# 3dv-casia/PanoVLM

Hardware: AMD Instinct MI355X
Metric: M residual+Jacobian evals/sec (point-to-plane, 64k pts/scan) (higher is better)
Workload: dtype f64

## Files before the change

panovlm_amd/csrc/pvlm_eval.hip:

```cpp
#include <algorithm>
#include <cmath>
#include <limits>

#include "pvlm_functors.h"
#include "pvlm_internal.h"

using namespace pvlm_dev;

#ifndef PVLM_NT_LOADS
#define PVLM_NT_LOADS 1
#endif
#ifndef PVLM_GLOBAL_LOADS
#define PVLM_GLOBAL_LOADS 1
#endif
typedef double pvlm_dbl2 __attribute__((ext_vector_type(2)));
#if PVLM_GLOBAL_LOADS
typedef const __attribute__((address_space(1))) pvlm_dbl2* pvlm_col_ptr;
#else
typedef const pvlm_dbl2* pvlm_col_ptr;
#endif
#ifndef PVLM_NT_LOADS_MATERIALISE
#define PVLM_NT_LOADS_MATERIALISE 0
#endif
__device__ __forceinline__ const double* at_byte(const double* base, unsigned bytes) {
  return reinterpret_cast<const double*>(reinterpret_cast<const char*>(base) + bytes);
}
template <bool NT>
__device__ __forceinline__ double2 stream_load2(const double* p) {
  pvlm_col_ptr q = (pvlm_col_ptr)(p);
  const pvlm_dbl2 v = NT ? __builtin_nontemporal_load(q) : *q;
  return make_double2(v.x, v.y);
}
struct pvlm_plane_args {
  const uint16_t* idx;
  const int64_t* pair_idx0;
  const int64_t* chunk_plane0;
  const double* tab;
  const double* const* pair_ptab;
  const int* order;
};
template <bool NT>
__device__ __forceinline__ unsigned stream_load_runs(const uint16_t* base, unsigned row) {
#if PVLM_GLOBAL_LOADS
  typedef const __attribute__((address_space(1))) unsigned* ptr;
#else
  typedef const unsigned* ptr;
#endif
  ptr q = (ptr)(reinterpret_cast<const char*>(base) + 2u * row);
  return NT ? __builtin_nontemporal_load(q) : *q;
}
template <bool NT>
__device__ __forceinline__ uint2 stream_load_words(const uint16_t* base, unsigned row) {
  typedef unsigned pvlm_u2 __attribute__((ext_vector_type(2)));
#if PVLM_GLOBAL_LOADS
  typedef const __attribute__((address_space(1))) pvlm_u2* ptr;
#else
  typedef const pvlm_u2* ptr;
#endif
  ptr q = (ptr)(reinterpret_cast<const char*>(base) + 4u * row);
  const pvlm_u2 v = NT ? __builtin_nontemporal_load(q) : *q;
  return make_uint2(v.x, v.y);
}
__device__ __forceinline__ double table_load(const double* base, unsigned bytes) {
#if PVLM_GLOBAL_LOADS
  typedef const __attribute__((address_space(1))) double* ptr;
#else
  typedef const double* ptr;
#endif
  return *(ptr)(reinterpret_cast<const char*>(base) + bytes);
}
#ifndef PVLM_NT_STORES
#define PVLM_NT_STORES 0
#endif
__device__ __forceinline__ void stream_store2(double2* p, double2 v) {
#if PVLM_NT_STORES
  pvlm_dbl2 w; w.x = v.x; w.y = v.y;
  __builtin_nontemporal_store(w, reinterpret_cast<pvlm_dbl2*>(p));
#else
  *p = v;
#endif
}
__device__ __forceinline__ void stream_store1(double* p, double v) {
#if PVLM_NT_STORES
  __builtin_nontemporal_store(v, p);
#else
  *p = v;
#endif
}


#ifndef PVLM_PREFETCH
#define PVLM_PREFETCH -1
#endif
#ifndef PVLM_FUSED_WAVES
#define PVLM_FUSED_WAVES 2
#endif
#ifndef PVLM_FUSED_WAVES_7COL
#define PVLM_FUSED_WAVES_7COL 4
#endif
#ifndef PVLM_FUSED_WAVES_WAVEFORM
#define PVLM_FUSED_WAVES_WAVEFORM 3
#endif

__global__ void k_pose_table(int n, const double* __restrict__ aa, const double* __restrict__ t, double* __restrict__ tab) {
  const int i = blockIdx.x * blockDim.x + threadIdx.x;
  if (i >= n) return;
  const double x = aa[3 * i], y = aa[3 * i + 1], z = aa[3 * i + 2];
  const double th2 = x * x + y * y + z * z;
  double* o = tab + (size_t)i * PVLM_POSE_TAB;
  double R[9];
  if (th2 > 2.220446049250313e-16) {
    const double th = sqrt(th2);
    const double wx = x / th, wy = y / th, wz = z / th;
    const double c = cos(th), s = sin(th), k = 1.0 - c;
    R[0] = c + wx * wx * k;      R[1] = wx * wy * k - wz * s; R[2] = wy * s + wx * wz * k;
    R[3] = wz * s + wx * wy * k; R[4] = c + wy * wy * k;      R[5] = -wx * s + wy * wz * k;
    R[6] = -wy * s + wx * wz * k; R[7] = wx * s + wy * wz * k; R[8] = c + wz * wz * k;
  } else {
    R[0] = 1; R[1] = -z; R[2] = y; R[3] = z; R[4] = 1; R[5] = -x; R[6] = -y; R[7] = x; R[8] = 1;
  }
  double A, B;
  if (th2 > 1e-6) {
    const double th = sqrt(th2);
    A = (1.0 - cos(th)) / th2;
    B = (th - sin(th)) / (th2 * th);
  } else {
    A = 0.5 - th2 * (1.0 / 24.0) + th2 * th2 * (1.0 / 720.0);
    B = (1.0 / 6.0) - th2 * (1.0 / 120.0) + th2 * th2 * (1.0 / 5040.0);
  }
  const double J[9] = {1.0 + B * (x * x - th2), -A * z + B * x * y,       A * y + B * x * z,
                       A * z + B * x * y,       1.0 + B * (y * y - th2), -A * x + B * y * z,
                       -A * y + B * x * z,      A * x + B * y * z,        1.0 + B * (z * z - th2)};
#pragma unroll
  for (int k = 0; k < 9; ++k) { o[k] = R[k]; o[9 + k] = J[k]; }
  o[18] = t[3 * i]; o[19] = t[3 * i + 1]; o[20] = t[3 * i + 2];
}

__global__ void k_pair_table(int P, const int* __restrict__ ref, const int* __restrict__ nei, int n_poses,
                             const double* __restrict__ pose, double* __restrict__ tab) {
  const int p = blockIdx.x * blockDim.x + threadIdx.x;
  if (p >= P) return;
  const int ir = ref[p], in = nei[p];
  double* o = tab + (size_t)p * PVLM_PAIR_TAB;
  if (ir >= n_poses || in >= n_poses) {
    for (int k = 0; k < PVLM_PAIR_TAB; ++k) o[k] = __longlong_as_double(0x7ff8000000000000LL);
    return;
  }
  const double* a = pose + (size_t)ir * PVLM_POSE_TAB;
  const double* b = pose + (size_t)in * PVLM_POSE_TAB;
  double R[9];
#pragma unroll
  for (int i = 0; i < 3; ++i)
#pragma unroll
    for (int j = 0; j < 3; ++j) R[i * 3 + j] = a[i * 3] * b[j * 3] + a[i * 3 + 1] * b[j * 3 + 1] + a[i * 3 + 2] * b[j * 3 + 2];
#pragma unroll
  for (int k = 0; k < 9; ++k) o[k] = R[k];
#pragma unroll
  for (int i = 0; i < 3; ++i) {
    o[9 + i] = a[18 + i] - (R[i * 3] * b[18] + R[i * 3 + 1] * b[19] + R[i * 3 + 2] * b[20]);
    o[12 + i] = a[18 + i];
  }
#pragma unroll
  for (int k = 0; k < 9; ++k) o[15 + k] = a[9 + k];
#pragma unroll
  for (int i = 0; i < 3; ++i)
#pragma unroll
    for (int j = 0; j < 3; ++j) o[24 + i * 3 + j] = -(R[i * 3] * b[9 + j] + R[i * 3 + 1] * b[9 + 3 + j] + R[i * 3 + 2] * b[9 + 6 + j]);
}

template <int KIND, bool NORM, int NCOLS>
__global__ __launch_bounds__(256) void k_eval_materialise(const double* const* __restrict__ pair_cols,
                                                          const int64_t* __restrict__ pair_stride,
                                                          const int64_t* __restrict__ out_start,
                                                          const int* __restrict__ blk_pair, const int* __restrict__ blk_chunk,
                                                          int chunk_rows, const double* __restrict__ pair_tab, double weight,
                                                          double* __restrict__ r_out, double* __restrict__ J_out, int blk0, int64_t row0) {
  const int bi = blockIdx.x + blk0;
  const int p = blk_pair[bi];
  const double* __restrict__ cols = pair_cols[p];
  const int64_t n_dev = pair_stride[p];
  const int64_t o0 = out_start[p] - row0;
  const int64_t len = out_start[p + 1] - out_start[p];
  const int64_t lo = (int64_t)blk_chunk[bi] * chunk_rows;
  const int64_t hi = min(len, lo + (int64_t)chunk_rows);
  double T[PVLM_PAIR_TAB];
#pragma unroll
  for (int k = 0; k < PVLM_PAIR_TAB; ++k) T[k] = pair_tab[(size_t)p * PVLM_PAIR_TAB + k];
  __shared__ __attribute__((aligned(16))) double stage[4][128 * 12];
  const int lane = threadIdx.x & 63, wv = threadIdx.x >> 6;
  const double* Jl = T + 15; const double* Mn = T + 24; const double* R = T;
  const int64_t n_it = (hi - lo + 511) / 512;
  for (int64_t it = 0; it < n_it; ++it) {
    const int64_t j = lo + it * 512 + 2 * (int64_t)threadIdx.x;
    if (j < hi) {
      double2 v[NCOLS];
#pragma unroll
      for (int c = 0; c < NCOLS; ++c) v[c] = stream_load2<PVLM_NT_LOADS_MATERIALISE != 0>(cols + (size_t)c * n_dev + j);
#pragma unroll
      for (int h = 0; h < 2; ++h) {
        if (j + h >= hi) break;
        double rec[NCOLS];
#pragma unroll
        for (int c = 0; c < NCOLS; ++c) rec[c] = h ? v[c].y : v[c].x;
        Wrench w;
        eval_wrench<KIND, NORM>(rec, T, weight, w);
        stream_store1(r_out + o0 + j + h, w.r);
        if (J_out) {
          double Jr[12];
#pragma unroll
          for (int k = 0; k < 3; ++k) {
            Jr[k] = w.c[0] * Jl[k] + w.c[1] * Jl[3 + k] + w.c[2] * Jl[6 + k];
            Jr[3 + k] = w.g[k];
            Jr[6 + k] = w.c[0] * Mn[k] + w.c[1] * Mn[3 + k] + w.c[2] * Mn[6 + k];
            Jr[9 + k] = -(w.g[0] * R[k] + w.g[1] * R[3 + k] + w.g[2] * R[6 + k]);
          }
          double2* dst = reinterpret_cast<double2*>(&stage[wv][(2 * lane + h) * 12]);
#pragma unroll
          for (int k = 0; k < 6; ++k) dst[k] = make_double2(Jr[2 * k], Jr[2 * k + 1]);
        }
      }
    }
    if (J_out) {
      __builtin_amdgcn_wave_barrier();
      const int64_t row0 = lo + it * 512 + (int64_t)wv * 128;
      const int64_t rows = min((int64_t)128, hi - row0);
      if (rows > 0) {
        double2* gdst = reinterpret_cast<double2*>(J_out + (size_t)(o0 + row0) * 12);
        const double2* src = reinterpret_cast<const double2*>(&stage[wv][0]);
        const int n2 = (int)rows * 6;
#pragma unroll
        for (int t = 0; t < 12; ++t) {
          const int e = t * 64 + lane;
          if (e < n2) stream_store2(gdst + e, src[e]);
        }
      }
      __builtin_amdgcn_wave_barrier();
    }
  }
}

template <int KIND, bool NORM, int NCOLS, int W>
__global__ __launch_bounds__(256) void k_eval_wrench(const double* const* __restrict__ pair_cols, const int64_t* __restrict__ pair_stride,
                                                     const int64_t* __restrict__ out_start, const int* __restrict__ blk_pair,
                                                     const int* __restrict__ blk_chunk, int chunk_rows, const double* __restrict__ pair_tab,
                                                     double weight, double* __restrict__ w_out, int blk0, int64_t row0) {
  const int bi = blockIdx.x + blk0;
  const int p = blk_pair[bi];
  const double* __restrict__ cols = pair_cols[p];
  const int64_t n_dev = pair_stride[p];
  const int64_t o0 = out_start[p] - row0;
  const int64_t len = out_start[p + 1] - out_start[p];
  const int64_t lo = (int64_t)blk_chunk[bi] * chunk_rows;
  const int64_t hi = min(len, lo + (int64_t)chunk_rows);
  double T[15];
#pragma unroll
  for (int k = 0; k < 15; ++k) T[k] = pair_tab[(size_t)p * PVLM_PAIR_TAB + k];
  __shared__ double stage[4][128 * W];
  const int lane = threadIdx.x & 63, wv = threadIdx.x >> 6;
  const int64_t n_it = (hi - lo + 511) / 512;
  for (int64_t it = 0; it < n_it; ++it) {
    const int64_t j = lo + it * 512 + 2 * (int64_t)threadIdx.x;
    if (j < hi) {
      double2 v[NCOLS];
#pragma unroll
      for (int c = 0; c < NCOLS; ++c) v[c] = stream_load2<PVLM_NT_LOADS_MATERIALISE != 0>(cols + (size_t)c * n_dev + j);
#pragma unroll
      for (int h = 0; h < 2; ++h) {
        if (j + h >= hi) break;
        double rec[NCOLS];
#pragma unroll
        for (int c = 0; c < NCOLS; ++c) rec[c] = h ? v[c].y : v[c].x;
        Wrench w;
        eval_wrench<KIND, NORM>(rec, T, weight, w);
        double* dst = &stage[wv][(2 * lane + h) * W];
        if (W == 7) { dst[0] = w.r; dst[1] = w.c[0]; dst[2] = w.c[1]; dst[3] = w.c[2]; dst[4] = w.g[0]; dst[5] = w.g[1]; dst[6] = w.g[2]; }
        else { dst[0] = w.r; dst[1] = w.g[0]; dst[2] = w.g[1]; dst[3] = w.g[2]; }
      }
    }
    __builtin_amdgcn_wave_barrier();
    const int64_t r0 = lo + it * 512 + (int64_t)wv * 128;
    const int64_t rows = min((int64_t)128, hi - r0);
    if (rows > 0) {
      double* g = w_out + (size_t)(o0 + r0) * W;
      const int n = (int)rows * W;
#pragma unroll
      for (int t = 0; t < 2 * W; ++t) {
        const int e = t * 64 + lane;
        if (e < n) stream_store1(g + e, stage[wv][e]);
      }
    }
    __builtin_amdgcn_wave_barrier();
  }
}

__device__ __forceinline__ double wave_sum(double x) {
#pragma unroll
  for (int off = 32; off > 0; off >>= 1) x += __shfl_down(x, off, 64);
  return x;
}

template <int KIND, bool NORM, int NCOLS, int LOSS>
__device__ __forceinline__ void accumulate_row(const double* rec, const double* T, double weight, double loss_a, double a2, double mh_a2, double* acc) {
  Wrench w;
  eval_wrench<KIND, NORM>(rec, T, weight, w);
  const double s = w.r * w.r;
  double rho1 = 1.0, half_rho = 0.5 * s;
  if (LOSS == PVLM_LOSS_HUBER) {
    const double rr = fabs(w.r);
    const bool out = s > a2;
    const double inv = fast_rcp(out ? rr : 1.0);
    rho1 = out ? fmax(std::numeric_limits<double>::min(), loss_a * inv) : 1.0;
    half_rho = out ? fma(loss_a, rr, mh_a2) : half_rho;
  }
  const double vv[6] = {w.c[0], w.c[1], w.c[2], w.g[0], w.g[1], w.g[2]};
  int q = 0;
#pragma unroll
  for (int a = 0; a < 6; ++a) {
    const double wa = rho1 * vv[a];
#pragma unroll
    for (int b = a; b < 6; ++b) acc[q++] += wa * vv[b];
    acc[21 + a] += wa * w.r;
  }
  acc[27] += half_rho;
}

template <int N>
__device__ __forceinline__ double wave_transpose_sum(const double (&a)[N], int lane) {
  static_assert(N <= 32, "at most 32 values");
  double v[32];
#pragma unroll
  for (int k = 0; k < 32; ++k) v[k] = k < N ? a[k] : 0.0;
#pragma unroll
  for (int half = 16; half >= 1; half >>= 1) {
    const bool up = (lane & (2 * half)) != 0;
#pragma unroll
    for (int k = 0; k < half; ++k) {
      const double keep = up ? v[half + k] : v[k];
      const double send = up ? v[k] : v[half + k];
      v[k] = keep + __shfl_xor(send, 2 * half, 64);
    }
  }
  return v[0] + __shfl_xor(v[0], 1, 64);
}

template <int KIND, bool NORM, int NCOLS, int LOSS, bool PR, bool PT>
__global__ __launch_bounds__(256, (NCOLS == 7 ? PVLM_FUSED_WAVES_7COL : PVLM_FUSED_WAVES)) void k_eval_fused(const double* const* __restrict__ pair_cols,
                                                    const int64_t* __restrict__ pair_stride,
                                                    const int64_t* __restrict__ out_start,
                                                    const int* __restrict__ blk_pair, const int* __restrict__ blk_chunk,
                                                    int chunk_rows, const double* __restrict__ pair_tab, double weight,
                                                    double loss_a, double* __restrict__ partials, pvlm_plane_args pr) {
  static_assert(!PR || NCOLS == 7, "plane runs: the 7-column kinds only");
  static_assert(!PT || PR, "the point table: on top of the plane runs only");
  const int slot = (PT && pr.order) ? pr.order[blockIdx.x] : (int)blockIdx.x;
  if (PT && slot < 0) return;
  constexpr int NS = PR ? 3 : NCOLS;
  const int p = blk_pair[slot];
  const double* __restrict__ cols = pair_cols[p];
  const int64_t n_dev = pair_stride[p];
  const int64_t len = out_start[p + 1] - out_start[p];
  const int64_t lo = (int64_t)blk_chunk[slot] * chunk_rows;
  const int64_t hi = min(len, lo + (int64_t)chunk_rows);
  double T[15];
#pragma unroll
  for (int k = 0; k < 15; ++k) T[k] = pair_tab[(size_t)p * PVLM_PAIR_TAB + k];
  double acc[PVLM_PARTIAL];
#pragma unroll
  for (int k = 0; k < PVLM_PARTIAL; ++k) acc[k] = 0.0;
  const double a2 = uniform_sgpr(loss_a * loss_a), mh_a2 = uniform_sgpr(-0.5 * a2);
  constexpr bool kPrefetch = !PT && (PVLM_PREFETCH >= 0 ? (PVLM_PREFETCH != 0) : (KIND == PVLM_POINT2PLANE_METER || KIND == PVLM_POINT2LINE_METER));
  const double* colb[NS];
#pragma unroll
  for (int c = 0; c < NS; ++c) colb[c] = PT ? pr.pair_ptab[p] + (size_t)c * PVLM_POINT_TAB_STRIDE : cols + (size_t)c * n_dev + lo;
  const uint16_t* runb = nullptr;
  const double* tabb = nullptr;
  if (PR) { runb = pr.idx + (PT ? 2 : 1) * (pr.pair_idx0[p] + lo); tabb = pr.tab + 4 * pr.chunk_plane0[slot]; }
  const unsigned span = hi > lo ? (unsigned)(hi - lo) : 0u;
  const unsigned span8 = 8u * span;
  unsigned o = 16u * threadIdx.x;
  double2 nx[NS];
  unsigned nx_runs = 0, nx_qs = 0;
  auto load_words = [&](unsigned row) {
    if (PT) { const uint2 w = stream_load_words<PVLM_NT_LOADS != 0>(runb, row); nx_runs = w.x; nx_qs = w.y; }
    else nx_runs = stream_load_runs<PVLM_NT_LOADS != 0>(runb, row);
  };
  if (PR && o < span8) load_words(o >> 3);
  if (kPrefetch && o < span8) {
#pragma unroll
    for (int c = 0; c < NS; ++c) nx[c] = stream_load2<PVLM_NT_LOADS != 0>(at_byte(colb[c], o));
  }
  for (; o < span8; o += 4096) {
    double2 v[NS];
    const unsigned runs = nx_runs, qs = nx_qs;
    const unsigned o_next = o + 4096 < span8 ? o + 4096 : o;
    if (kPrefetch) {
#pragma unroll
      for (int c = 0; c < NS; ++c) v[c] = nx[c];
      if (PR) load_words(o_next >> 3);
      if (o + 4096 < span8) {
#pragma unroll
        for (int c = 0; c < NS; ++c) nx[c] = stream_load2<PVLM_NT_LOADS != 0>(at_byte(colb[c], o + 4096));
      }
    } else {
#ifdef PVLM_EXP_SKIP
#pragma unroll
      for (int c = 0; c < NS; ++c) v[c] = *reinterpret_cast<const double2*>(colb[c < NS - PVLM_EXP_SKIP ? c : 0] + (o >> 3));
#else
      if (PT) {
        const unsigned q0 = 8u * (qs & 0xffffu), q1 = 8u * (qs >> 16);
#pragma unroll
        for (int c = 0; c < NS; ++c) v[c] = make_double2(table_load(colb[c], q0), table_load(colb[c], q1));
      } else {
#pragma unroll
        for (int c = 0; c < NS; ++c) v[c] = stream_load2<PVLM_NT_LOADS != 0>(at_byte(colb[c], o));
      }
#endif
    }
    double2 pl[2][2];
    if (PR) {
#pragma unroll
      for (int h = 0; h < 2; ++h) {
        const unsigned at = 32u * (h ? runs >> 16 : runs & 0xffffu);
        pl[h][0] = stream_load2<false>(at_byte(tabb, at));
        pl[h][1] = stream_load2<false>(at_byte(tabb, at + 16u));
      }
      if (!kPrefetch) load_words(o_next >> 3);
    }
#pragma unroll
    for (int h = 0; h < 2; ++h) {
      if (o + 8u * h >= span8) break;
      double rec[NCOLS];
#pragma unroll
      for (int c = 0; c < NS; ++c) rec[c] = h ? v[c].y : v[c].x;
      if (PR) { rec[3] = pl[h][0].x; rec[4] = pl[h][0].y; rec[5] = pl[h][1].x; rec[6] = pl[h][1].y; }
      accumulate_row<KIND, NORM, NCOLS, LOSS>(rec, T, weight, loss_a, a2, mh_a2, acc);
    }
  }
  __shared__ double red[4][PVLM_PARTIAL];
  const int lane = threadIdx.x & 63, wv = threadIdx.x >> 6;
  {
    const double s = wave_transpose_sum<PVLM_PARTIAL>(acc, lane);
    if (!(lane & 1) && (lane >> 1) < PVLM_PARTIAL) red[wv][lane >> 1] = s;
  }
  __syncthreads();
  if (threadIdx.x < PVLM_PARTIAL)
    partials[(size_t)slot * PVLM_PARTIAL + threadIdx.x] =
        ((red[0][threadIdx.x] + red[1][threadIdx.x]) + red[2][threadIdx.x]) + red[3][threadIdx.x];
}

template <int KIND, bool NORM, int NCOLS, int LOSS, bool PR>
__global__ __launch_bounds__(256, PVLM_FUSED_WAVES_WAVEFORM) void k_eval_fused_wave(const double* const* __restrict__ pair_cols,
                                                    const int64_t* __restrict__ pair_stride,
                                                    const int64_t* __restrict__ out_start,
                                                    const int* __restrict__ blk_pair, const int* __restrict__ blk_chunk,
                                                    int chunk_rows, int n_units, const double* __restrict__ pair_tab, double weight,
                                                    double loss_a, double* __restrict__ partials, pvlm_plane_args pr) {
  static_assert(!PR || NCOLS == 7, "plane runs: the 7-column kinds only");
  constexpr int NS = PR ? 3 : NCOLS;
  const int unit = __builtin_amdgcn_readfirstlane(blockIdx.x * 4 + (threadIdx.x >> 6)), lane = threadIdx.x & 63;
  if (unit >= n_units) return;
  const int p = blk_pair[unit];
  const double* __restrict__ cols = pair_cols[p];
  const int64_t n_dev = pair_stride[p];
  const int64_t len = out_start[p + 1] - out_start[p];
  const int64_t lo = (int64_t)blk_chunk[unit] * chunk_rows;
  const int64_t hi = min(len, lo + (int64_t)chunk_rows);
  double T[15];
#pragma unroll
  for (int k = 0; k < 15; ++k) T[k] = pair_tab[(size_t)p * PVLM_PAIR_TAB + k];
  double acc[PVLM_PARTIAL];
#pragma unroll
  for (int k = 0; k < PVLM_PARTIAL; ++k) acc[k] = 0.0;
  const double a2 = uniform_sgpr(loss_a * loss_a), mh_a2 = uniform_sgpr(-0.5 * a2);
  const double* colb[NS];
#pragma unroll
  for (int c = 0; c < NS; ++c) colb[c] = cols + (size_t)c * n_dev + lo;
  const uint16_t* runb = nullptr;
  const double* tabb = nullptr;
  if (PR) { runb = pr.idx + pr.pair_idx0[p] + lo; tabb = pr.tab + 4 * pr.chunk_plane0[unit]; }
  const unsigned span = hi > lo ? (unsigned)(hi - lo) : 0u;
  unsigned nx_runs = 0;
  if (PR && 2u * lane < span) nx_runs = stream_load_runs<PVLM_NT_LOADS != 0>(runb, 2u * lane);
  for (unsigned j = 2u * lane; j < span; j += 128) {
    double2 v[NS];
#pragma unroll
    for (int c = 0; c < NS; ++c) v[c] = stream_load2<PVLM_NT_LOADS != 0>(at_byte(colb[c], 8u * j));
    double2 pl[2][2];
    if (PR) {
      const unsigned runs = nx_runs;
#pragma unroll
      for (int h = 0; h < 2; ++h) {
        const unsigned at = 32u * (h ? runs >> 16 : runs & 0xffffu);
        pl[h][0] = stream_load2<false>(at_byte(tabb, at));
        pl[h][1] = stream_load2<false>(at_byte(tabb, at + 16u));
      }
      nx_runs = stream_load_runs<PVLM_NT_LOADS != 0>(runb, j + 128 < span ? j + 128 : j);
    }
#pragma unroll
    for (int h = 0; h < 2; ++h) {
      if (j + h >= span) break;
      double rec[NCOLS];
#pragma unroll
      for (int c = 0; c < NS; ++c) rec[c] = h ? v[c].y : v[c].x;
      if (PR) { rec[3] = pl[h][0].x; rec[4] = pl[h][0].y; rec[5] = pl[h][1].x; rec[6] = pl[h][1].y; }
      accumulate_row<KIND, NORM, NCOLS, LOSS>(rec, T, weight, loss_a, a2, mh_a2, acc);
    }
  }
  const double mine = wave_transpose_sum<PVLM_PARTIAL>(acc, lane);
  if (!(lane & 1) && (lane >> 1) < PVLM_PARTIAL) partials[(size_t)unit * PVLM_PARTIAL + (lane >> 1)] = mine;
}

__global__ __launch_bounds__(128) void k_pair_epilogue(int P, const int* __restrict__ pair_blk_start,
                                                       const double* __restrict__ partials,
                                                       const double* __restrict__ pair_tab, double* __restrict__ out) {
  const int p = blockIdx.x;
  __shared__ double S[6][6], gv[6], Dr[6][6], Dn[6][6], cost;
  __shared__ double tot[PVLM_PARTIAL];
  const int t = threadIdx.x;
  if (t < PVLM_PARTIAL) {
    double s = 0.0;
    for (int b = pair_blk_start[p]; b < pair_blk_start[p + 1]; ++b) s += partials[(size_t)b * PVLM_PARTIAL + t];
    tot[t] = s;
  }
  if (t < 36) {
    const int i = t / 6, j = t % 6;
    const double* T = pair_tab + (size_t)p * PVLM_PAIR_TAB;
    double dr = 0.0, dn = 0.0;
    if (i < 3 && j < 3) { dr = T[15 + i * 3 + j]; dn = T[24 + i * 3 + j]; }
    else if (i >= 3 && j >= 3) { dr = (i == j) ? 1.0 : 0.0; dn = -T[(i - 3) * 3 + (j - 3)]; }
    Dr[i][j] = dr; Dn[i][j] = dn;
  }
  __syncthreads();
  if (t < 36) {
    const int i = t / 6, j = t % 6;
    const int a = i < j ? i : j, b = i < j ? j : i;
    S[i][j] = tot[a * 6 - a * (a - 1) / 2 + (b - a)];
  }
  if (t < 6) gv[t] = tot[21 + t];
  if (t == 0) cost = tot[27];
  __syncthreads();
  double* o = out + (size_t)p * PVLM_PAIR_BLOCK;
  if (t < 108) {
    const int blk = t / 36, i = (t % 36) / 6, j = t % 6;
    const double(*L)[6] = (blk == 2) ? Dn : Dr;
    const double(*Rm)[6] = (blk == 0) ? Dr : Dn;
    double s = 0.0;
    for (int a = 0; a < 6; ++a) {
      double u = 0.0;
      for (int b = 0; b < 6; ++b) u += S[a][b] * Rm[b][j];
      s += L[a][i] * u;
    }
    o[t] = s;
  } else if (t < 120) {
    const int i = (t - 108) % 6;
    const double(*L)[6] = (t < 114) ? Dr : Dn;
    double s = 0.0;
    for (int a = 0; a < 6; ++a) s += L[a][i] * gv[a];
    o[t] = s;
  } else if (t == 120) {
    o[120] = cost;
  }
}

__global__ void k_neq_gather(int n_poses, int n_upairs, const int* __restrict__ diag_off, const int* __restrict__ diag_items,
                             const int* __restrict__ off_off, const int* __restrict__ off_items,
                             const double* __restrict__ pair_blocks, int P, int zero_first, double* __restrict__ packed) {
  const int b = blockIdx.x, t = threadIdx.x;
  double* Hd = packed;
  double* Ho = packed + (size_t)n_poses * 36;
  double* g = Ho + (size_t)n_upairs * 36;
  double* cost = g + (size_t)n_poses * 6;
  if (b < n_poses) {
    if (t < 42) {
      double s = 0.0;
      for (int k = diag_off[b]; k < diag_off[b + 1]; ++k) {
        const int it = diag_items[k];
        const double* pb = pair_blocks + (size_t)(it >> 1) * PVLM_PAIR_BLOCK;
        const int role = it & 1;
        s += (t < 36) ? pb[(role ? 72 : 0) + t] : pb[108 + (role ? 6 : 0) + (t - 36)];
      }
      double* dst = (t < 36) ? &Hd[(size_t)b * 36 + t] : &g[(size_t)b * 6 + (t - 36)];
      *dst = zero_first ? s : (*dst + s);
    }
  } else if (b < n_poses + n_upairs) {
    const int u = b - n_poses;
    if (t < 36) {
      const int i = t / 6, j = t % 6;
      double s = 0.0;
      for (int k = off_off[u]; k < off_off[u + 1]; ++k) {
        const int it = off_items[k];
        const double* pb = pair_blocks + (size_t)(it >> 1) * PVLM_PAIR_BLOCK + 36;
        s += (it & 1) ? pb[j * 6 + i] : pb[t];
      }
      double* dst = &Ho[(size_t)u * 36 + t];
      *dst = zero_first ? s : (*dst + s);
    }
  } else {
    __shared__ double red[256];
    double s = 0.0;
    for (int p = t; p < P; p += 256) s += pair_blocks[(size_t)p * PVLM_PAIR_BLOCK + 120];
    red[t] = s;
    __syncthreads();
    for (int w = 128; w > 0; w >>= 1) { if (t < w) red[t] += red[t + w]; __syncthreads(); }
    if (t == 0) *cost = zero_first ? red[0] : (*cost + red[0]);
  }
}

static pvlm_status ensure_pose_cap(pvlm_ctx* ctx, int n) {
  if (n <= ctx->cap_poses) return PVLM_OK;
  if (ctx->capturing) { PVLM_SET_ERR(ctx, "pose table would grow inside a graph capture (run the step once before pvlm_graph_begin)"); return PVLM_ERR_STATE; }
  PVLM_TRY_SYNC(ctx);
  pvlm_i_free(ctx, ctx->d_aa); pvlm_i_free(ctx, ctx->d_t); pvlm_i_free(ctx, ctx->d_pose_tab);
  ctx->d_aa = ctx->d_t = ctx->d_pose_tab = nullptr;
  ctx->cap_poses = 0;
  pvlm_status st;
  if ((st = pvlm_i_alloc(ctx, &ctx->d_aa, (size_t)n * 3))) return st;
  if ((st = pvlm_i_alloc(ctx, &ctx->d_t, (size_t)n * 3))) return st;
  if ((st = pvlm_i_alloc(ctx, &ctx->d_pose_tab, (size_t)n * PVLM_POSE_TAB))) return st;
  ctx->cap_poses = n;
  return PVLM_OK;
}

static pvlm_status pose_table_launch(pvlm_ctx* ctx, int n, const double* d_aa, const double* d_t) {
  if (n > 0) {
    hipLaunchKernelGGL(k_pose_table, dim3((n + 63) / 64), dim3(64), 0, ctx->stream, n, d_aa, d_t, ctx->d_pose_tab);
    PVLM_HIP(ctx, hipGetLastError());
// ... 389 lines not shown
```

panovlm_amd/csrc/pvlm_functors.h:

```cpp
#pragma once
#include <hip/hip_runtime.h>

#include "pvlm_internal.h"

namespace pvlm_dev {

struct Wrench { double r; double c[3]; double g[3]; };

__device__ __forceinline__ double dot3(const double* a, const double* b) { return a[0] * b[0] + a[1] * b[1] + a[2] * b[2]; }
__device__ __forceinline__ void cross3(const double* a, const double* b, double* o) {
  o[0] = a[1] * b[2] - a[2] * b[1]; o[1] = a[2] * b[0] - a[0] * b[2]; o[2] = a[0] * b[1] - a[1] * b[0];
}


__device__ __forceinline__ double fast_rcp(double x) {
  const double r = __builtin_amdgcn_rcp(x);
  return fma(r, fma(-x, r, 1.0), r);
}
__device__ __forceinline__ double fast_rsqrt(double x) {
  const double r = __builtin_amdgcn_rsq(x);
  return fma(r, fma(-x * r, 0.5 * r, 0.5), r);
}
__device__ __forceinline__ double horner10_sconst(double u, double c0, double c1, double c2, double c3, double c4, double c5, double c6, double c7,
                                                  double c8, double c9) {
#if defined(__HIP_DEVICE_COMPILE__)
  double p;
  asm("v_mov_b64 %0, %2\n\t"
      "v_fma_f64 %0, %0, %1, %3\n\t"
      "v_fma_f64 %0, %0, %1, %4\n\t"
      "v_fma_f64 %0, %0, %1, %5\n\t"
      "v_fma_f64 %0, %0, %1, %6\n\t"
      "v_fma_f64 %0, %0, %1, %7\n\t"
      "v_fma_f64 %0, %0, %1, %8\n\t"
      "v_fma_f64 %0, %0, %1, %9\n\t"
      "v_fma_f64 %0, %0, %1, %10\n\t"
      "v_fma_f64 %0, %0, %1, %11\n\t"
      "v_fma_f64 %0, %0, %1, 1.0"
      : "=&v"(p)
      : "v"(u), "s"(c0), "s"(c1), "s"(c2), "s"(c3), "s"(c4), "s"(c5), "s"(c6), "s"(c7), "s"(c8), "s"(c9));
  return p;
#else
  double p = fma(c0, u, c1);
  for (double c : {c2, c3, c4, c5, c6, c7, c8, c9, 1.0}) p = fma(p, u, c);
  return p;
#endif
}
__device__ __forceinline__ double uniform_sgpr(double x) {
#if defined(__HIP_DEVICE_COMPILE__)
  const unsigned long long b = (unsigned long long)__double_as_longlong(x);
  const unsigned lo = (unsigned)__builtin_amdgcn_readfirstlane((int)(unsigned)b), hi = (unsigned)__builtin_amdgcn_readfirstlane((int)(unsigned)(b >> 32));
  return __longlong_as_double((long long)(((unsigned long long)hi << 32) | lo));
#else
  return x;
#endif
}
__device__ __forceinline__ double atan_small(double t) {
  const double u = t * t;
  return t * horner10_sconst(u, 2.11272689568591313e-02, -4.34739031566048761e-02, 5.68812005923421543e-02, -6.64019012732186553e-02,
                             7.68994845277858746e-02, -9.09077271667437237e-02, 1.11111061650365134e-01, -1.42857141805968924e-01,
                             1.99999999988503901e-01, -3.33333333333284132e-01);
}
__device__ __forceinline__ double atan2_octants(double y, double x) {
  const double ax = fabs(x);
  const double mn = fmin(y, ax), mx = fmax(y, ax);
  const double a = mn * fast_rcp(mx);
  const bool big = a > 0.41421356237309503;
  const double red = (a - 1.0) * fast_rcp(a + 1.0);
  double r = atan_small(big ? red : a);
  r = big ? r + 0.78539816339744830962 : r;
  r = (y > ax) ? 1.57079632679489661923 - r : r;
  return (x < 0.0) ? 3.14159265358979323846 - r : r;
}
__device__ __forceinline__ double atan2_pos(double y, double x) {
  if (__all(y <= 0.41421356237309503 * x)) return atan_small(y * fast_rcp(x));
  return atan2_octants(y, x);
}
__device__ __forceinline__ double atan2_pos_grad(double y, double x, bool live, double& inv_h2) {
  const double h2 = fma(x, x, y * y);
  double r;
  if (__all(y <= 0.41421356237309503 * x)) {
    const double R = live ? fast_rcp(x * h2) : 0.0;
    inv_h2 = x * R;
    r = atan_small(y * (h2 * R));
  } else {
    inv_h2 = live ? fast_rcp(h2) : 0.0;
    r = live ? atan2_octants(y, x) : 0.0;
  }
  return r;
}

__device__ __forceinline__ bool angle_between(const double* v1, const double* v2, double& r, double* g1, double* g2) {
  const double d = dot3(v1, v2);
  const double q1 = dot3(v1, v1), q2 = dot3(v2, v2);
  const double n1 = sqrt(q1), n2 = sqrt(q2);
  const double c = d / (n1 * n2);
  if (c >= 1.0) { r = 0.0; return false; }
  if (c <= -1.0) { r = M_PI; return false; }
  double w[3], a1[3], a2[3];
  cross3(v1, v2, w);
  const double nw = sqrt(dot3(w, w));
  if (!(nw > 0.0)) { r = d < 0.0 ? M_PI : 0.0; return false; }
  r = atan2_pos(nw, d);
  cross3(v1, w, a1);
  cross3(v2, w, a2);
  const double k1 = 1.0 / (q1 * nw), k2 = -1.0 / (q2 * nw);
#pragma unroll
  for (int k = 0; k < 3; ++k) { g1[k] = k1 * a1[k]; g2[k] = k2 * a2[k]; }
  return true;
}

template <bool NORM>
__device__ __forceinline__ bool normalized_angle(const double* P, const double* Pp, double& r, double* gP, double* gPp) {
  if (NORM) {
    const double nu2 = dot3(Pp, Pp);
    const double nu = sqrt(nu2);
    const double ratio = (nu - 1.0) / nu;
    double v1[3], v2[3], g1[3], g2[3];
#pragma unroll
    for (int k = 0; k < 3; ++k) { const double ck = ratio * Pp[k]; v1[k] = Pp[k] - ck; v2[k] = P[k] - ck; }
    if (!angle_between(v1, v2, r, g1, g2)) return false;
    double gc[3] = {-(g1[0] + g2[0]), -(g1[1] + g2[1]), -(g1[2] + g2[2])};
    const double s = dot3(Pp, gc) / (nu2 * nu);
#pragma unroll
    for (int k = 0; k < 3; ++k) { gP[k] = g2[k]; gPp[k] = g1[k] + ratio * gc[k] + s * Pp[k]; }
    return true;
  }
  return angle_between(P, Pp, r, gP, gPp);
}

template <int KIND, bool NORM>
__device__ __forceinline__ void residual_grad(const double* P, const double* rec, double w, double& r, double* g) {
  g[0] = g[1] = g[2] = 0.0;
  r = 0.0;
  if (KIND == PVLM_POINT2PLANE_METER) {
    const double* n = rec + 3;
    const double sd = n[0] * P[0] + n[1] * P[1] + n[2] * P[2] + n[3];
    const double s = sd < 0.0 ? -w : w;
    r = s * sd;
    g[0] = s * n[0]; g[1] = s * n[1]; g[2] = s * n[2];
  } else if (KIND == PVLM_POINT2PLANE_ANGLE && NORM) {
    const double* n = rec + 3;
    const double dd = n[3];
    const double sd = n[0] * P[0] + n[1] * P[1] + n[2] * P[2] + dd;
    const double dis = fabs(sd);
    const double u[3] = {P[0] - (sd - dd) * n[0], P[1] - (sd - dd) * n[1], P[2] - (sd - dd) * n[2]};
    const double q2 = dot3(u, u);
    const double nu2 = q2 + dd * dd;
    const double inv_nu = fast_rsqrt(nu2);
    const double invq = q2 > 0.0 ? fast_rsqrt(q2) : 0.0;
    const double q = q2 * invq, nu = nu2 * inv_nu;
    const double X = fma(-sd, dd, nu), Y = dis * q;
    const bool live = dis >= 1e-3;
    double AD = q * nu, BD = dis * dd * fma(-sd, nu, dd) * (invq * inv_nu);
#if defined(__HIP_DEVICE_COMPILE__)
    asm volatile("" : "+v"(AD), "+v"(BD));
#endif
    double k0;
    r = atan2_pos_grad(Y, X, live, k0);
    const double A = copysign(AD * k0, sd);
    const double B = BD * k0;
#pragma unroll
    for (int k = 0; k < 3; ++k) g[k] = A * n[k] + B * u[k];
  } else if (KIND == PVLM_POINT2PLANE_ANGLE) {
    const double* n = rec + 3;
    const double sd = n[0] * P[0] + n[1] * P[1] + n[2] * P[2] + n[3];
    const double s = sd < 0.0 ? -1.0 : 1.0;
    const double dis = s * sd;
    if (dis < 1e-3) return;
    double Pp[3] = {P[0] - dis * n[0], P[1] - dis * n[1], P[2] - dis * n[2]};
    double sig = 1.0;
    if (fabs(n[0] * Pp[0] + n[1] * Pp[1] + n[2] * Pp[2] + n[3]) > 1e-4) {
      Pp[0] = P[0] + dis * n[0]; Pp[1] = P[1] + dis * n[1]; Pp[2] = P[2] + dis * n[2];
      sig = -1.0;
    }
    double gP[3], gPp[3];
    if (!normalized_angle<NORM>(P, Pp, r, gP, gPp)) return;
    const double t = sig * s * dot3(n, gPp);
#pragma unroll
    for (int k = 0; k < 3; ++k) g[k] = gP[k] + gPp[k] - t * n[k];
  } else if (KIND == PVLM_POINT2LINE_METER) {
    const double* A = rec + 3; const double* d = rec + 6;
    const double dd = d[0] * d[0] + d[1] * d[1] + d[2] * d[2];
    const double k = (d[0] * (P[0] - A[0]) + d[1] * (P[1] - A[1]) + d[2] * (P[2] - A[2])) / dd;
    const double e[3] = {k * d[0] + A[0] - P[0], k * d[1] + A[1] - P[1], k * d[2] + A[2] - P[2]};
    const double dist = sqrt(dot3(e, e));
    r = w * dist;
    const double q = dot3(d, e) / dd;
    const double wi = w / dist;
#pragma unroll
    for (int kk = 0; kk < 3; ++kk) g[kk] = wi * (q * d[kk] - e[kk]);
  } else if (KIND == PVLM_POINT2LINE_ANGLE) {
    const double* A = rec + 3; const double* d = rec + 6;
    const double k = d[0] * (P[0] - A[0]) + d[1] * (P[1] - A[1]) + d[2] * (P[2] - A[2]);
    const double Pp[3] = {k * d[0] + A[0], k * d[1] + A[1], k * d[2] + A[2]};
    const double e[3] = {P[0] - Pp[0], P[1] - Pp[1], P[2] - Pp[2]};
    const double dis = sqrt(dot3(e, e));
    if (dis < 1e-3) return;
    double gP[3], gPp[3];
    if (!normalized_angle<NORM>(P, Pp, r, gP, gPp)) return;
    const double t = dot3(d, gPp);
#pragma unroll
    for (int kk = 0; kk < 3; ++kk) g[kk] = gP[kk] + t * d[kk];
  }
}

template <int KIND, bool NORM>
__device__ __forceinline__ void eval_wrench(const double* rec, const double* T, double w, Wrench& out) {
  const double* R = T; const double* trn = T + 9; const double* trw = T + 12;
  auto chain = [&](const double* p, double* o) {
    o[0] = R[0] * p[0] + R[1] * p[1] + R[2] * p[2] + trn[0];
    o[1] = R[3] * p[0] + R[4] * p[1] + R[5] * p[2] + trn[1];
    o[2] = R[6] * p[0] + R[7] * p[1] + R[8] * p[2] + trn[2];
  };
  if (KIND <= PVLM_POINT2LINE_ANGLE) {
    double P[3];
    chain(rec, P);
    residual_grad<KIND, NORM>(P, rec, w, out.r, out.g);
    const double m[3] = {P[0] - trw[0], P[1] - trw[1], P[2] - trw[2]};
    cross3(m, out.g, out.c);
  } else if (KIND == PVLM_PLANE2PLANE_GLOBAL) {
    const double* ni = rec; const double wk = rec[9];
    double a[3], b[3], nrm[3];
    chain(rec + 3, a);
    chain(rec + 6, b);
    cross3(a, b, nrm);
    out.r = 0.0;
#pragma unroll
    for (int k = 0; k < 3; ++k) { out.c[k] = 0.0; out.g[k] = 0.0; }
    const double dp = dot3(ni, nrm);
    const double s = dp < 0.0 ? -1.0 : 1.0;
    const double q1 = dot3(ni, ni), q2 = dot3(nrm, nrm);
    const double c = s * dp / (sqrt(q1) * sqrt(q2));
    if (c >= 1.0) return;
    double wv[3], nxw[3];
    cross3(ni, nrm, wv);
    const double nw = sqrt(dot3(wv, wv));
    if (!(nw > 0.0)) return;
    out.r = wk * atan2_pos(nw, s * dp);
    cross3(nrm, wv, nxw);
    const double kg = -wk * s / (q2 * nw);
    double gn[3], ga[3], gb[3], ca[3], cb[3];
#pragma unroll
    for (int k = 0; k < 3; ++k) gn[k] = kg * nxw[k];
    cross3(b, gn, ga);
    cross3(gn, a, gb);
    const double ma[3] = {a[0] - trw[0], a[1] - trw[1], a[2] - trw[2]};
    const double mb[3] = {b[0] - trw[0], b[1] - trw[1], b[2] - trw[2]};
    cross3(ma, ga, ca);
    cross3(mb, gb, cb);
#pragma unroll
    for (int k = 0; k < 3; ++k) { out.c[k] = ca[k] + cb[k]; out.g[k] = ga[k] + gb[k]; }
  } else {
    const double* n = rec; const double* mr = rec + 7; const double ang = rec[10]; const double wk = rec[11];
    double mc[3];
    chain(rec + 4, mc);
    out.r = 0.0;
#pragma unroll
    for (int k = 0; k < 3; ++k) { out.c[k] = 0.0; out.g[k] = 0.0; }
    const double sd = n[0] * mc[0] + n[1] * mc[1] + n[2] * mc[2] + n[3];
    const double s = sd < 0.0 ? -1.0 : 1.0;
    const double dis = s * sd;
    double np[3] = {mc[0] - dis * n[0], mc[1] - dis * n[1], mc[2] - dis * n[2]};
    double sig = 1.0;
    if (fabs(n[0] * np[0] + n[1] * np[1] + n[2] * np[2] + n[3]) > 1e-4) {
      np[0] = mc[0] + dis * n[0]; np[1] = mc[1] + dis * n[1]; np[2] = mc[2] + dis * n[2];
      sig = -1.0;
    }
    double cur, g1[3], g2[3];
    const bool smooth = angle_between(np, mr, cur, g1, g2);
    if (cur < ang) return;
    out.r = wk * (cur - ang);
    if (!smooth) return;
    const double t = sig * s * dot3(n, g1);
    double g[3];
#pragma unroll
    for (int k = 0; k < 3; ++k) g[k] = wk * (g1[k] - t * n[k]);
    const double m[3] = {mc[0] - trw[0], mc[1] - trw[1], mc[2] - trw[2]};
    cross3(m, g, out.c);
#pragma unroll
    for (int k = 0; k < 3; ++k) out.g[k] = g[k];
  }
}

}
```

Before: 140,500.

## Add wave-uniform Huber inlier fast path and truncated atan polynomial tier

Accumulation of the normal-equation outer product now checks, via a wave ballot, whether any lane is a Huber outlier. If none is, it takes an unweighted path without the reciprocal and the rho multiplies, and the accumulation uses explicit FMAs. Separately, when every lane in the wave has a very small atan argument (32*y <= x), only the last four Horner terms of the atan polynomial are evaluated. This trims FP64 work in common cases but adds ballot and branch overhead. For the tiny case the truncated polynomial relies on the higher-order terms being negligible.

```diff
diff --git a/panovlm_amd/csrc/pvlm_eval.hip b/panovlm_amd/csrc/pvlm_eval.hip
--- a/panovlm_amd/csrc/pvlm_eval.hip
+++ b/panovlm_amd/csrc/pvlm_eval.hip
@@ -299,29 +299,47 @@
   return x;
 }
 
+#ifndef PVLM_HUBER_SLOT
+#define PVLM_HUBER_SLOT 1
+#endif
+
+template <bool WEIGHTED>
+__device__ __forceinline__ void accumulate_outer(const double (&vv)[6], double r, double rho1, double half_rho, double* acc) {
+  int q = 0;
+#pragma unroll
+  for (int a = 0; a < 6; ++a) {
+    const double wa = WEIGHTED ? rho1 * vv[a] : vv[a];
+#pragma unroll
+    for (int b = a; b < 6; ++b, ++q) acc[q] = fma(wa, vv[b], acc[q]);
+    acc[21 + a] = fma(wa, r, acc[21 + a]);
+  }
+  acc[27] += half_rho;
+}
+
 template <int KIND, bool NORM, int NCOLS, int LOSS>
 __device__ __forceinline__ void accumulate_row(const double* rec, const double* T, double weight, double loss_a, double a2, double mh_a2, double* acc) {
   Wrench w;
   eval_wrench<KIND, NORM>(rec, T, weight, w);
   const double s = w.r * w.r;
-  double rho1 = 1.0, half_rho = 0.5 * s;
-  if (LOSS == PVLM_LOSS_HUBER) {
+  const double vv[6] = {w.c[0], w.c[1], w.c[2], w.g[0], w.g[1], w.g[2]};
+  if (LOSS != PVLM_LOSS_HUBER) { accumulate_outer<false>(vv, w.r, 1.0, 0.5 * s, acc); return; }
+  const bool out = s > a2;
+  auto general = [&]() {
     const double rr = fabs(w.r);
-    const bool out = s > a2;
     const double inv = fast_rcp(out ? rr : 1.0);
-    rho1 = out ? fmax(std::numeric_limits<double>::min(), loss_a * inv) : 1.0;
-    half_rho = out ? fma(loss_a, rr, mh_a2) : half_rho;
-  }
-  const double vv[6] = {w.c[0], w.c[1], w.c[2], w.g[0], w.g[1], w.g[2]};
-  int q = 0;
-#pragma unroll
-  for (int a = 0; a < 6; ++a) {
-    const double wa = rho1 * vv[a];
-#pragma unroll
-    for (int b = a; b < 6; ++b) acc[q++] += wa * vv[b];
-    acc[21 + a] += wa * w.r;
-  }
-  acc[27] += half_rho;
+    const double rho1 = out ? fmax(std::numeric_limits<double>::min(), loss_a * inv) : 1.0;
+    const double half_rho = out ? fma(loss_a, rr, mh_a2) : 0.5 * s;
+    accumulate_outer<true>(vv, w.r, rho1, half_rho, acc);
+  };
+#if PVLM_HUBER_SLOT && defined(__HIP_DEVICE_COMPILE__)
+  const unsigned long long outliers = __ballot(out);
+  unsigned long long none = outliers;
+  asm("" : "+s"(none));
+  if (outliers != 0) general();
+  if (none == 0) accumulate_outer<false>(vv, w.r, 1.0, 0.5 * s, acc);
+#else
+  general();
+#endif
 }
 
 template <int N>
diff --git a/panovlm_amd/csrc/pvlm_functors.h b/panovlm_amd/csrc/pvlm_functors.h
--- a/panovlm_amd/csrc/pvlm_functors.h
+++ b/panovlm_amd/csrc/pvlm_functors.h
@@ -21,10 +21,26 @@
   const double r = __builtin_amdgcn_rsq(x);
   return fma(r, fma(-x * r, 0.5 * r, 0.5), r);
 }
+#ifndef PVLM_ATAN_TIER
+#define PVLM_ATAN_TIER 1
+#endif
+#define PVLM_ATAN_TIER_ENTRY 6
+template <int ENTRY = 0>
 __device__ __forceinline__ double horner10_sconst(double u, double c0, double c1, double c2, double c3, double c4, double c5, double c6, double c7,
                                                   double c8, double c9) {
+  static_assert(ENTRY == 0 || ENTRY == 6, "entry points with a statement below");
 #if defined(__HIP_DEVICE_COMPILE__)
   double p;
+  if (ENTRY == 6) {
+    asm("v_mov_b64 %0, %2\n\t"
+        "v_fma_f64 %0, %0, %1, %3\n\t"
+        "v_fma_f64 %0, %0, %1, %4\n\t"
+        "v_fma_f64 %0, %0, %1, %5\n\t"
+        "v_fma_f64 %0, %0, %1, 1.0"
+        : "=&v"(p)
+        : "v"(u), "s"(c6), "s"(c7), "s"(c8), "s"(c9));
+    return p;
+  }
   asm("v_mov_b64 %0, %2\n\t"
       "v_fma_f64 %0, %0, %1, %3\n\t"
       "v_fma_f64 %0, %0, %1, %4\n\t"
@@ -40,8 +56,9 @@
       : "v"(u), "s"(c0), "s"(c1), "s"(c2), "s"(c3), "s"(c4), "s"(c5), "s"(c6), "s"(c7), "s"(c8), "s"(c9));
   return p;
 #else
-  double p = fma(c0, u, c1);
-  for (double c : {c2, c3, c4, c5, c6, c7, c8, c9, 1.0}) p = fma(p, u, c);
+  const double c[11] = {c0, c1, c2, c3, c4, c5, c6, c7, c8, c9, 1.0};
+  double p = c[ENTRY];
+  for (int k = ENTRY + 1; k < 11; ++k) p = fma(p, u, c[k]);
   return p;
 #endif
 }
@@ -54,11 +71,12 @@
   return x;
 #endif
 }
+template <int ENTRY = 0>
 __device__ __forceinline__ double atan_small(double t) {
   const double u = t * t;
-  return t * horner10_sconst(u, 2.11272689568591313e-02, -4.34739031566048761e-02, 5.68812005923421543e-02, -6.64019012732186553e-02,
-                             7.68994845277858746e-02, -9.09077271667437237e-02, 1.11111061650365134e-01, -1.42857141805968924e-01,
-                             1.99999999988503901e-01, -3.33333333333284132e-01);
+  return t * horner10_sconst<ENTRY>(u, 2.11272689568591313e-02, -4.34739031566048761e-02, 5.68812005923421543e-02, -6.64019012732186553e-02,
+                                    7.68994845277858746e-02, -9.09077271667437237e-02, 1.11111061650365134e-01, -1.42857141805968924e-01,
+                                    1.99999999988503901e-01, -3.33333333333284132e-01);
 }
 __device__ __forceinline__ double atan2_octants(double y, double x) {
   const double ax = fabs(x);
@@ -72,16 +90,22 @@
   return (x < 0.0) ? 3.14159265358979323846 - r : r;
 }
 __device__ __forceinline__ double atan2_pos(double y, double x) {
-  if (__all(y <= 0.41421356237309503 * x)) return atan_small(y * fast_rcp(x));
+  const bool tiny = PVLM_ATAN_TIER && __all(32.0 * y <= x);
+  if (tiny || __all(y <= 0.41421356237309503 * x)) {
+    const double t = y * fast_rcp(x);
+    return tiny ? atan_small<PVLM_ATAN_TIER_ENTRY>(t) : atan_small(t);
+  }
   return atan2_octants(y, x);
 }
 __device__ __forceinline__ double atan2_pos_grad(double y, double x, bool live, double& inv_h2) {
   const double h2 = fma(x, x, y * y);
   double r;
-  if (__all(y <= 0.41421356237309503 * x)) {
+  const bool tiny = PVLM_ATAN_TIER && __all(32.0 * y <= x);
+  if (tiny || __all(y <= 0.41421356237309503 * x)) {
     const double R = live ? fast_rcp(x * h2) : 0.0;
     inv_h2 = x * R;
-    r = atan_small(y * (h2 * R));
+    const double t = y * (h2 * R);
+    r = tiny ? atan_small<PVLM_ATAN_TIER_ENTRY>(t) : atan_small(t);
   } else {
     inv_h2 = live ? fast_rcp(h2) : 0.0;
     r = live ? atan2_octants(y, x) : 0.0;
```

Measured after the change: 142,800, median of 6. 1.7% higher.
